# PlasmaControl/spectrogram-enhancement

Hardware: AMD Instinct MI355X
Metric: spectrograms/s (STFT+VAE-denoise fwd) at 1/2/4/8 GPUs; PSNR vs CPU ref (higher is better)
Workload: dtype fp16; 1 GPU; BASELINE config 5 per GPU: end-to-end STFT -> SVD -> autoencoder-denoise inference stream, 16,512-sample fp16 shots -> specgr 128x128 (256 hann / hop 128) -> denoiseSignal default -> 3-layer conv AE (16/32/64, 5x5) fp16 forward -> fp16 reconstructions (32,768 B per shot); shots_per_launch=2048, samples=16512, stft_dtype=fp32, svd_dtype=fp32 (fp64 small algebra), ae_dtype=fp16, parallelism=shot-sharded x1, streams_per_gpu=2

## Files before the change

### spectrogram-enhancement_amd/csrc/conv_rows.hip

```cpp
#include <hip/hip_runtime.h>

#include <algorithm>
#include <cstdint>
#include <string>
#include <type_traits>

#include "lds_dma.hpp"
#include "specenh.h"
#include "runtime.hpp"
#include "wave.hpp"

namespace specenh {

namespace {

typedef _Float16 f16x8 __attribute__((ext_vector_type(8)));
typedef __bf16 bf16x8 __attribute__((ext_vector_type(8)));
typedef float f32x4 __attribute__((ext_vector_type(4)));

template <typename T>
__device__ __forceinline__ f32x4 mfma(const uint4& a, const uint4& b, f32x4 acc) {
  if constexpr (__is_same(T, _Float16))
    return __builtin_amdgcn_mfma_f32_16x16x32_f16(__builtin_bit_cast(f16x8, a),
                                                  __builtin_bit_cast(f16x8, b), acc, 0, 0, 0);
  else
    return __builtin_amdgcn_mfma_f32_16x16x32_bf16(__builtin_bit_cast(bf16x8, a),
                                                   __builtin_bit_cast(bf16x8, b), acc, 0, 0, 0);
}

template <typename T>
__device__ __forceinline__ uint32_t pack2(float lo, float hi) {
  typedef float f2 __attribute__((ext_vector_type(2)));
  typedef T t2 __attribute__((ext_vector_type(2)));
  return __builtin_bit_cast(uint32_t, __builtin_convertvector(f2{lo, hi}, t2));
}


__device__ __forceinline__ float max_pair(float v) {
  const float o = __int_as_float(__builtin_amdgcn_update_dpp(0, __float_as_int(v), 0xB1, 0xF, 0xF, true));
  return fmaxf(v, o);
}

template <int CIN, int COUT, int W, int K = 5>
struct RC {
  static constexpr int NWIN = W / 16;
  static constexpr int NNB = COUT / 16;
  static constexpr int WAVES = NWIN * NNB;
  static constexpr int THREADS = 64 * WAVES;
  static constexpr int PIX = CIN * 2;
  static constexpr int ROWB = (W + 4) * PIX;
  static constexpr int RING = 8;
  static constexpr int LDS = RING * ROWB;
  static constexpr int NW = CIN == 16 ? 13 : K * K;
  static_assert(K == 5 || (CIN == 32 && (K == 3 || K == 5)), "kernel size");
  static constexpr int CPP = CIN / 8;
  static constexpr int CHUNKS = W * CPP;
  static constexpr int WPR = CHUNKS / 64;
  static constexpr int DMA_WAVES = 2 * WPR;
  static_assert(WAVES == 8 && CHUNKS % 64 == 0 && DMA_WAVES <= WAVES, "shape");
  static constexpr int WPE = CIN == 16 || K == 3 ? 4 : 2;
};

struct CRArgs {
  const void* x;
  const void* w;
  const float* b;
  void* out;
  int N, H;
  int lgb;
};

template <typename T, int CIN, int COUT, int W, int K = 5>
__global__ __launch_bounds__((RC<CIN, COUT, W, K>::THREADS))
__attribute__((amdgpu_waves_per_eu(RC<CIN, COUT, W, K>::WPE)))
void conv_rows_pool_kernel(CRArgs a) {
  using C = RC<CIN, COUT, W, K>;
  extern __shared__ __attribute__((aligned(16))) unsigned char ring[];
  const int tid = threadIdx.x, lane = tid & 63;
  const int wv = __builtin_amdgcn_readfirstlane(tid >> 6);
  const int m = lane & 15, kg = lane >> 4;
  const int wx = wv % C::NWIN, nb = wv / C::NWIN;
  const int x0 = 16 * wx;
  const int H = a.H, SPI = H / 2 + 1;
  const int G = gridDim.x;
  const int nimg = ((int)a.N - (int)blockIdx.x + G - 1) / G;
  const int S = nimg * SPI + 1;

  {
    uint4* z = reinterpret_cast<uint4*>(ring);
    for (int e = tid; e < C::LDS / 16; e += C::THREADS) z[e] = uint4{0u, 0u, 0u, 0u};
  }

  uint4 wf[C::NW];
  {
    const T* __restrict__ Wg = reinterpret_cast<const T*>(a.w);
    const int co = 16 * nb + m;
    auto tap = [&](int ky, int kx, int c8) {
      return *reinterpret_cast<const uint4*>(Wg + ((co * K + ky) * K + kx) * CIN + c8);
    };
    if constexpr (CIN == 32) {
#pragma unroll
      for (int t = 0; t < K * K; ++t) wf[t] = tap(t / K, t % K, 8 * kg);
    } else {
      const int hi = kg >> 1, c8 = 8 * (kg & 1);
#pragma unroll
      for (int ky = 0; ky < 5; ++ky) {
        wf[ky] = tap(ky, hi, c8);
        wf[5 + ky] = tap(ky, 2 + hi, c8);
      }
      wf[10] = tap(hi, 4, c8);
      wf[11] = tap(2 + hi, 4, c8);
      wf[12] = hi ? uint4{0u, 0u, 0u, 0u} : tap(4, 4, c8);
    }
  }
  const f32x4 bias = f32x4{a.b[16 * nb + 4 * kg], a.b[16 * nb + 4 * kg + 1],
                           a.b[16 * nb + 4 * kg + 2], a.b[16 * nb + 4 * kg + 3]};

  int boff[CIN == 32 ? K : 1];
  int foff = 0, foffw = 0, fo0 = 0;
  if constexpr (CIN == 32) {
#pragma unroll
    for (int kx = 0; kx < K; ++kx) {
      const int ps = x0 + m + kx + 2 - K / 2;
      boff[kx] = ps * 64 + 16 * (kg ^ ((ps >> 1) & 3));
    }
  } else {
    boff[0] = (x0 + m + (kg >> 1)) * 32 + 16 * (kg & 1);
    const int fo = (x0 + m + 4) * 32 + 16 * (kg & 1);
    fo0 = fo;
    foff = fo + (kg >> 1) * C::ROWB;
    foffw = fo - (kg >> 1) * 7 * C::ROWB;
  }

  const T* __restrict__ X = reinterpret_cast<const T*>(a.x);
  const bool dma_wave = wv < C::DMA_WAVES;
  int dsrc = 0, ddst = 0;
  if (dma_wave) {
    const int c = (wv % C::WPR) * 64 + lane;
    const int ps = 2 + c / C::CPP, gs = c % C::CPP;
    const int g = CIN == 32 ? (gs ^ ((ps >> 1) & 3)) : gs;
    dsrc = (ps - 2) * CIN + 8 * g;
    ddst = 2 * C::PIX + (wv % C::WPR) * 1024;
  }
  auto stage_at = [&](int s, int il, int q) -> bool {
    if (!dma_wave) return false;
    const int r = 2 * q + wv / C::WPR;
    unsigned char* dst = ring + ((2 * s + wv / C::WPR) & 7) * C::ROWB + ddst;
    if (s < S && il < nimg && r < H) {
      const long long n = (long long)blockIdx.x + (long long)il * G;
      lds_dma16_s(X + ((n * H + r) * W) * CIN, 2u * dsrc, dst);
      return true;
    }
    *reinterpret_cast<uint4*>(dst + 16 * lane) = uint4{0u, 0u, 0u, 0u};
    return false;
  };
  auto stage = [&](int s) { return stage_at(s, s / SPI, s - (s / SPI) * SPI); };
  __syncthreads();
  stage(0);
  stage(1);
  stage(2);
  asm volatile("s_waitcnt vmcnt(0)" ::: "memory");
  lds_barrier();

  f32x4 acc[6];
#pragma unroll
  for (int i = 0; i < 6; ++i) acc[i] = bias;
  T* __restrict__ O = reinterpret_cast<T*>(a.out);
  const int PW = W / 2, PHh = H / 2;

  int ilA = -1, qA = SPI - 2, ilC = 0, qC = 0, ilS = 3 / SPI, qS = 3 - (3 / SPI) * SPI;
  auto adv = [&](int& il, int& q) {
    if (++q == SPI) { q = 0; ++il; }
  };
  auto step = [&](auto ic, const int s) {
    constexpr int I = decltype(ic)::value;
    auto slot = [](int d) { return (2 * I + d + 12) % 6; };
    {
      f32x4& r0 = acc[slot(-4)];
      f32x4& r1 = acc[slot(-3)];
      {
        const int il = ilA, q = qA;
        if (il >= 0 && il < nimg && q < PHh) {
          float v[4];
#pragma unroll
          for (int i = 0; i < 4; ++i) v[i] = fmaxf(max_pair(fmaxf(r0[i], r1[i])), 0.f);
          const long long n = (long long)blockIdx.x + (long long)il * G;
          const long long o = ((n * PHh + q) * PW + (x0 + m) / 2) * COUT + 16 * nb + 4 * kg;
          *reinterpret_cast<uint2*>(O + o) = uint2{pack2<T>(v[0], v[1]), pack2<T>(v[2], v[3])};
        }
      }
      r0 = bias;
      r1 = bias;
    }
    const bool issued = stage_at(s + 3, ilS, qS);
    const int il = ilC, q = qC;
    if (il < nimg && 2 * q < H) {
      constexpr int NB = CIN == 32 ? K : 3;
      uint4 bf[2][NB];
#pragma unroll
      for (int j = 0; j < 2; ++j) {
        const int rs = (2 * s + j) & 7;
        const unsigned char* rb = ring + rs * C::ROWB;
        if constexpr (CIN == 32) {
#pragma unroll
          for (int kx = 0; kx < K; ++kx) bf[j][kx] = *reinterpret_cast<const uint4*>(rb + boff[kx]);
        } else {
          bf[j][0] = *reinterpret_cast<const uint4*>(rb + boff[0]);
          bf[j][1] = *reinterpret_cast<const uint4*>(rb + boff[0] + 64);
          bf[j][2] = *reinterpret_cast<const uint4*>(rb + (rs == 7 ? foffw : foff));
        }
      }
      uint4 bT = uint4{0u, 0u, 0u, 0u};
      if constexpr (CIN == 16) {
        if (q == 0) {
          bT = *reinterpret_cast<const uint4*>(ring + ((2 * s) & 7) * C::ROWB + fo0);
          if (kg < 2) bT = uint4{0u, 0u, 0u, 0u};
        }
      }
      __builtin_amdgcn_sched_barrier(0);
#pragma unroll
      for (int j = 0; j < 2; ++j) {
        if constexpr (CIN == 32) {
#pragma unroll
          for (int kx = 0; kx < K; ++kx)
#pragma unroll
            for (int ky = 0; ky < K; ++ky) {
              f32x4& ac = acc[slot(j + K / 2 - ky)];
              ac = mfma<T>(wf[ky * K + kx], bf[j][kx], ac);
            }
        } else {
#pragma unroll
          for (int ky = 0; ky < 5; ++ky) {
            f32x4& ac = acc[slot(j + 2 - ky)];
            ac = mfma<T>(wf[ky], bf[j][0], ac);
          }
#pragma unroll
          for (int ky = 0; ky < 5; ++ky) {
            f32x4& ac = acc[slot(j + 2 - ky)];
            ac = mfma<T>(wf[5 + ky], bf[j][1], ac);
          }
          acc[slot(j + 2)] = mfma<T>(wf[10], bf[j][2], acc[slot(j + 2)]);
          acc[slot(j)] = mfma<T>(wf[11], bf[j][2], acc[slot(j)]);
          acc[slot(j - 2)] = mfma<T>(wf[12], bf[j][2], acc[slot(j - 2)]);
          if (j == 0 && q == 0) acc[slot(1)] = mfma<T>(wf[10], bT, acc[slot(1)]);
        }
      }
    }
    if (issued) asm volatile("s_waitcnt vmcnt(1)" ::: "memory");
    else asm volatile("s_waitcnt vmcnt(0)" ::: "memory");
    adv(ilA, qA);
    adv(ilC, qC);
    adv(ilS, qS);
    lds_barrier();
  };
  int s = 0;
  for (; s + 3 <= S; s += 3) {
    step(std::integral_constant<int, 0>{}, s);
    step(std::integral_constant<int, 1>{}, s + 1);
    step(std::integral_constant<int, 2>{}, s + 2);
  }
  if (s < S) step(std::integral_constant<int, 0>{}, s);
  if (s + 1 < S) step(std::integral_constant<int, 1>{}, s + 1);
}

template <typename T, int CIN, int COUT, int W, int K = 5>
hipError_t launch_rows(const CRArgs& a, hipStream_t st) {
  using C = RC<CIN, COUT, W, K>;
  const void* k = reinterpret_cast<const void*>(&conv_rows_pool_kernel<T, CIN, COUT, W, K>);
  static int per_cu[64] = {};
  int dev = 0;
  hipError_t e = hipGetDevice(&dev);
  if (e != hipSuccess) return e;
  if (dev < 0 || dev >= 64) dev = 0;
  if (per_cu[dev] == 0) {
    int pc = 0;
    e = hipOccupancyMaxActiveBlocksPerMultiprocessor(&pc, k, C::THREADS, C::LDS);
    if (e != hipSuccess) return e;
    per_cu[dev] = std::max(1, pc);
  }
  const long long grid = std::min<long long>(a.N, (long long)per_cu[dev] * device_cus());
  SPECENH_LAUNCH((conv_rows_pool_kernel<T, CIN, COUT, W, K>), dim3((unsigned)grid),
                 dim3(C::THREADS), C::LDS, st, a);
  return hipGetLastError();
}

template <int CO, int W>
struct TC {
  static constexpr int CI = 64;
  static constexpr int NWIN = W / 16, NNB = CO / 16;
  static constexpr int WAVES = NWIN * NNB;
  static constexpr int THREADS = 64 * WAVES;
  static constexpr int ROWB = (W + 2) * CI * 2;
  static constexpr int RING = 8;
  static constexpr int LDS = RING * ROWB;
  static constexpr int DMA_WAVES = W * CI * 2 / 1024;
  static_assert(WAVES == 4 && DMA_WAVES <= WAVES, "shape");
};

__device__ __forceinline__ constexpr int tky(int py, int dy) { return 2 * dy + 3 - py; }
__device__ __forceinline__ constexpr bool ttap(int ph, int dy, int dx) {
  return tky(ph >> 1, dy) >= 0 && tky(ph >> 1, dy) < 5 && tky(ph & 1, dx) >= 0 &&
         tky(ph & 1, dx) < 5;
}

template <typename T>
__device__ __forceinline__ uint32_t relu2(uint32_t p) {
  if constexpr (__is_same(T, _Float16)) {
    typedef _Float16 h2 __attribute__((ext_vector_type(2)));
    const h2 z = h2{(_Float16)0.f, (_Float16)0.f};
    return __builtin_bit_cast(uint32_t, __builtin_elementwise_max(__builtin_bit_cast(h2, p), z));
  } else {
    typedef short s2 __attribute__((ext_vector_type(2)));
    const uint32_t neg = __builtin_bit_cast(uint32_t, __builtin_bit_cast(s2, p) >> (short)15);
    return p & ~neg;
  }
}
template <typename T>
__device__ __forceinline__ uint2 relu_pack4(const f32x4& v) {
  return uint2{relu2<T>(pack2<T>(v[0], v[1])), relu2<T>(pack2<T>(v[2], v[3]))};
}

template <typename T, int CO, int W, int LEAD>
__global__ __launch_bounds__((TC<CO, W>::THREADS)) __attribute__((amdgpu_waves_per_eu(2)))
void convt_rows_kernel(CRArgs a) {
  static_assert(LEAD >= 1 && LEAD <= 4, "8-row ring: positions g .. g + 3 + LEAD live");
  using C = TC<CO, W>;
  extern __shared__ __attribute__((aligned(16))) unsigned char ring[];
  const int tid = threadIdx.x, lane = tid & 63;
  const int wv = __builtin_amdgcn_readfirstlane(tid >> 6);
  const int m = lane & 15, kg = lane >> 4;
  const int wx = wv % C::NWIN, nb = wv / C::NWIN;
  const int H = a.H, lgb = a.lgb, HB = H >> lgb, bmask = (1 << lgb) - 1;
  const int SPI = HB + (lgb ? 2 : 1);
  const int G = gridDim.x;
  const int nimg = (((int)a.N << lgb) - (int)blockIdx.x + G - 1) / G;
  const int S = nimg * SPI;

  {
    uint4* z = reinterpret_cast<uint4*>(ring);
    for (int e = tid; e < C::LDS / 16; e += C::THREADS) z[e] = uint4{0u, 0u, 0u, 0u};
  }
  uint4 wf[50];
  {
    const T* __restrict__ Wg = reinterpret_cast<const T*>(a.w);
    int u = 0;
#pragma unroll
    for (int ph = 0; ph < 4; ++ph)
#pragma unroll
      for (int dy = -1; dy <= 1; ++dy)
#pragma unroll
        for (int dx = -1; dx <= 1; ++dx) {
          if (!ttap(ph, dy, dx)) continue;
#pragma unroll
          for (int kh = 0; kh < 2; ++kh)
            wf[u++] = *reinterpret_cast<const uint4*>(
                Wg + (((16 * nb + m) * 5 + tky(ph >> 1, dy)) * 5 + tky(ph & 1, dx)) * 64 +
                32 * kh + 8 * kg);
        }
  }
  const f32x4 bias = f32x4{a.b[16 * nb + 4 * kg], a.b[16 * nb + 4 * kg + 1],
                           a.b[16 * nb + 4 * kg + 2], a.b[16 * nb + 4 * kg + 3]};
  resident_loads_landed();
  int xo[3];
#pragma unroll
  for (int dx = -1; dx <= 1; ++dx) {
    const int ps = 16 * wx + m + dx + 1;
    xo[dx + 1] = ps * 128 + 16 * (kg ^ (ps & 7));
  }
  const T* __restrict__ X = reinterpret_cast<const T*>(a.x);
  const bool dma_wave = wv < C::DMA_WAVES;
  int dsrc = 0;
  if (dma_wave) {
    const int c = 64 * wv + lane;
    const int ps = 1 + c / 8, gs = c & 7;
    dsrc = (ps - 1) * 64 + 8 * (gs ^ (ps & 7));
  }
  auto stage_at = [&](int p, int il, int q) -> bool {
    if (!dma_wave) return false;
    unsigned char* dst = ring + (p & 7) * C::ROWB + 128 + 1024 * wv;
    const int v = (int)blockIdx.x + il * G;
    const int r = (v & bmask) * HB + q - 1;
    if (il < nimg && r >= 0 && r < H) {
      const long long n = (long long)(v >> lgb);
      lds_dma16_s(X + ((n * H + r) * W) * 64, 2u * dsrc, dst);
      return true;
    }
    *reinterpret_cast<uint4*>(dst + 16 * lane) = uint4{0u, 0u, 0u, 0u};
    return false;
  };
  auto stage = [&](int p) -> bool {
    const int il = p / SPI;
    return stage_at(p, il, p - il * SPI);
  };
  __syncthreads();
#pragma unroll
  for (int p = 0; p < 3 + LEAD; ++p) stage(p);
  asm volatile("s_waitcnt vmcnt(0)" ::: "memory");
  lds_barrier();

  T* __restrict__ O = reinterpret_cast<T*>(a.out);
  const int OW = 2 * W;
  uint2 pk[4];
  long long po = 0;
  bool held = false;
  int vmn = 0;
  int mk[LEAD + 1];
#pragma unroll
  for (int i = 0; i <= LEAD; ++i) mk[i] = -1;
  auto store_held = [&]() {
    if (held) {
#pragma unroll
      for (int ph = 0; ph < 4; ++ph)
        gstore8(O + po + ((ph >> 1) * OW + (ph & 1)) * CO, pk[ph]);
      vmn += 4;
    }
  };
  int il = 0, s = 0;
  int ilp = (3 + LEAD) / SPI, sp = 3 + LEAD - ilp * SPI;
  for (int g = 0; g < S; ++g) {
    store_held();
    held = false;
    mk[LEAD] = stage_at(g + 3 + LEAD, ilp, sp) ? ++vmn : -1;
    if (s < HB) {
      f32x4 acc[4] = {bias, bias, bias, bias};
      int u0[4] = {0, 8, 20, 32};
#pragma unroll
      for (int dy = -1; dy <= 1; ++dy) {
        const unsigned char* src = ring + ((g + 1 + dy) & 7) * C::ROWB;
#pragma unroll
        for (int dx = -1; dx <= 1; ++dx) {
          const uint4 b0 = *reinterpret_cast<const uint4*>(src + xo[dx + 1]);
          const uint4 b1 = *reinterpret_cast<const uint4*>(src + (xo[dx + 1] ^ 64));
#pragma unroll
          for (int ph = 0; ph < 4; ++ph)
// ... 1075 lines not shown
  produce(1, 1 / SPI, 1 % SPI);
  lds_barrier();

  f32x4 acc[6];
#pragma unroll
  for (int i = 0; i < 6; ++i) acc[i] = bias2_ld();
  T* __restrict__ O = reinterpret_cast<T*>(a.out);
  const int PW = 32, PHh = H / 2;
  int c_1 = 0, c_2 = 0;
  auto fdiv = [](int x, int d) { return x >= 0 ? x / d : -((-x + d - 1) / d); };
  int ilA = fdiv(-2, SPI), qA = -2 - ilA * SPI;
  int qC = 0;
  int ilB = 2 / SPI, qB = 2 - ilB * SPI;
  int ilD = (32 + wv) / PPI, rD = 32 + wv - ilD * PPI;
  auto adv = [](int& il, int& q, int by, int per) {
    q += by;
    if (q >= per) { q -= per; ++il; }
  };

  auto step = [&](auto ic, const int s) {
    constexpr int I = decltype(ic)::value;
    auto slot = [](int d) { return (2 * I + d + 12) % 6; };
    int ns = 0;
    {
      f32x4& r0 = acc[slot(-4)];
      f32x4& r1 = acc[slot(-3)];
      {
        const int il = ilA, q = qA;
        if (il >= 0 && il < nimg && q < PHh) {
          ns = 1;
          float v[4];
#pragma unroll
          for (int i = 0; i < 4; ++i) v[i] = fmaxf(max_pair(fmaxf(r0[i], r1[i])), 0.f);
          const long long n = (long long)blockIdx.x + (long long)il * G;
          const long long o = ((n * PHh + q) * PW + (x0 + m) / 2) * 32 + 16 * nb + 4 * kg;
          *reinterpret_cast<uint2*>(O + o) = uint2{pack2<T>(v[0], v[1]), pack2<T>(v[2], v[3])};
        }
      }
      const f32x4 bias = bias2_ld();
      r0 = bias;
      r1 = bias;
    }
    const int nd = wv < 4 ? stage1_at(4 * s + 32 + wv, ilD, rD - 2) : 0;
    shift1(4 * s + 16);
    const int q = qC;
    auto conv2_rows = [&]() {
#pragma unroll
    for (int j = 0; j < 2; ++j) {
      const int rs = (2 * s + j) & 7;
      const unsigned char* rb = ring + rs * C::ROWB;
      const uint4 b0 = *reinterpret_cast<const uint4*>(rb + boff);
      const uint4 b2 = *reinterpret_cast<const uint4*>(rb + boff + 64);
      uint4 bF = *reinterpret_cast<const uint4*>(rb + (rs == 7 ? foffw : foff));
      if (j == 1 && q == SPI - 1) bF = uint4{0u, 0u, 0u, 0u};
#pragma unroll
      for (int ky = 0; ky < 5; ++ky) {
        f32x4& ac = acc[slot(j + 2 - ky)];
        ac = mfma<T>(wf[ky], b0, ac);
      }
#pragma unroll
      for (int ky = 0; ky < 5; ++ky) {
        f32x4& ac = acc[slot(j + 2 - ky)];
        ac = mfma<T>(wf[5 + ky], b2, ac);
      }
      acc[slot(j + 2)] = mfma<T>(wf[10], bF, acc[slot(j + 2)]);
      acc[slot(j)] = mfma<T>(wf[11], bF, acc[slot(j)]);
      acc[slot(j - 2)] = mfma<T>(wf[12], bF, acc[slot(j - 2)]);
      if (j == 0) {
        uint4 bT = *reinterpret_cast<const uint4*>(ring + ((2 * s) & 7) * C::ROWB + fo);
        if (kg < 2 || q != 0) bT = uint4{0u, 0u, 0u, 0u};
        acc[slot(1)] = mfma<T>(wf[10], bT, acc[slot(1)]);
      }
    }
    };
    if (SPECENH_ENC2_STAGGER && wv >= 4) {
      conv2_rows();
      produce(s + 2, ilB, qB);
    } else {
      produce(s + 2, ilB, qB);
      conv2_rows();
    }
    if (wv < 4) {
      const int younger = c_2 + c_1 + ns + nd;
      if (younger >= 6) {
        asm volatile("s_waitcnt vmcnt(6)" ::: "memory");
      } else switch (younger) {
        case 0: asm volatile("s_waitcnt vmcnt(0)" ::: "memory"); break;
        case 1: asm volatile("s_waitcnt vmcnt(1)" ::: "memory"); break;
        case 2: asm volatile("s_waitcnt vmcnt(2)" ::: "memory"); break;
        case 3: asm volatile("s_waitcnt vmcnt(3)" ::: "memory"); break;
        case 4: asm volatile("s_waitcnt vmcnt(4)" ::: "memory"); break;
        case 5: asm volatile("s_waitcnt vmcnt(5)" ::: "memory"); break;
        default: asm volatile("s_waitcnt vmcnt(6)" ::: "memory"); break;
      }
    }
    c_2 = c_1;
    c_1 = ns + nd;
    adv(ilA, qA, 1, SPI);
    qC = qC + 1 == SPI ? 0 : qC + 1;
    adv(ilB, qB, 1, SPI);
    adv(ilD, rD, 4, PPI);
    lds_barrier();
  };
  int s = 0;
  for (; s + 3 <= S; s += 3) {
    step(std::integral_constant<int, 0>{}, s);
    step(std::integral_constant<int, 1>{}, s + 1);
    step(std::integral_constant<int, 2>{}, s + 2);
  }
  if (s < S) step(std::integral_constant<int, 0>{}, s);
  if (s + 1 < S) step(std::integral_constant<int, 1>{}, s + 1);
}

constexpr int E2LDS = RC<16, 32, 64>::LDS + E2RROWS * E2ROW * 4 + 48 * 4;

template <typename T, int WPE>
hipError_t launch_enc2_wpe(const E2Args& a, hipStream_t st) {
  const void* k = reinterpret_cast<const void*>(&enc2_rows_kernel<T, WPE>);
  static int per_cu[64] = {};
  int dev = 0;
  hipError_t e = hipGetDevice(&dev);
  if (e != hipSuccess) return e;
  if (dev < 0 || dev >= 64) dev = 0;
  if (per_cu[dev] == 0) {
    int pc = 0;
    e = hipOccupancyMaxActiveBlocksPerMultiprocessor(&pc, k, 512, E2LDS);
    if (e != hipSuccess) return e;
    per_cu[dev] = std::max(1, pc);
  }
  const long long grid = std::min<long long>(a.N, (long long)per_cu[dev] * device_cus());
  SPECENH_LAUNCH((enc2_rows_kernel<T, WPE>), dim3((unsigned)grid), dim3(512), E2LDS, st, a);
  return hipGetLastError();
}

template <typename T>
hipError_t launch_enc2(const E2Args& a, hipStream_t st) {
  return variant(V_ENC2_WPE2) ? launch_enc2_wpe<T, 2>(a, st) : launch_enc2_wpe<T, 4>(a, st);
}

}

int conv_rows_pool(int dtype, const void* x, int N, int H, int W, int CI, const void* w,
                   const float* b, int CO, int K, void* out, hipStream_t st, bool* launched) {
  *launched = false;
  if (variant(V_CONV_NO_ROWS) != 0 || N <= 0 || H < 2 || (H & 1) || !b) return SPECENH_OK;
  if ((long long)N * H * W * CI >= (1ll << 31)) return SPECENH_OK;
  CRArgs a{};
  a.x = x; a.w = w; a.b = b; a.out = out; a.N = N; a.H = H;
  hipError_t e = hipSuccess;
  const bool f16 = dtype == SPECENH_DTYPE_F16;
  if (dtype != SPECENH_DTYPE_F16 && dtype != SPECENH_DTYPE_BF16) return SPECENH_OK;
  if (CI == 16 && CO == 32 && W == 64 && K == 5)
    e = f16 ? launch_rows<_Float16, 16, 32, 64>(a, st) : launch_rows<__bf16, 16, 32, 64>(a, st);
  else if (CI == 32 && CO == 64 && W == 32 && K == 5)
    e = f16 ? launch_rows<_Float16, 32, 64, 32>(a, st) : launch_rows<__bf16, 32, 64, 32>(a, st);
  else if (CI == 32 && CO == 32 && W == 64 && K == 5)
    e = f16 ? launch_rows<_Float16, 32, 32, 64>(a, st) : launch_rows<__bf16, 32, 32, 64>(a, st);
  else if (CI == 32 && CO == 32 && W == 64 && K == 3)
    e = f16 ? launch_rows<_Float16, 32, 32, 64, 3>(a, st) : launch_rows<__bf16, 32, 32, 64, 3>(a, st);
  else
    return SPECENH_OK;
  if (e != hipSuccess) return set_error(SPECENH_EHIP, std::string("conv_rows: ") + hipGetErrorString(e));
  *launched = true;
  return SPECENH_OK;
}

}

namespace specenh {

int convt_rows(int dtype, const void* x, int N, int H, int W, int CI, const void* w,
               const float* b, int CO, int K, void* out, hipStream_t st, bool* launched) {
  *launched = false;
  if (variant(V_CONVT_NO_ROWS) != 0 || N <= 0 || H <= 0 || !b) return SPECENH_OK;
  if (dtype != SPECENH_DTYPE_F16 && dtype != SPECENH_DTYPE_BF16) return SPECENH_OK;
  if ((long long)N * 4 * H * W * CO >= (1ll << 31)) return SPECENH_OK;
  CRArgs a{};
  a.x = x; a.w = w; a.b = b; a.out = out; a.N = N; a.H = H;
  const bool f16 = dtype == SPECENH_DTYPE_F16;
  hipError_t e;
  if (CI == 32) {
    if (CO != 32 || W != 32) return SPECENH_OK;
    if (K == 3) e = f16 ? launch_convt_rows32<_Float16, 32, 32, 3>(a, st) : launch_convt_rows32<__bf16, 32, 32, 3>(a, st);
    else if (K == 5) e = f16 ? launch_convt_rows32<_Float16, 32, 32, 5>(a, st) : launch_convt_rows32<__bf16, 32, 32, 5>(a, st);
    else if (K == 7) e = f16 ? launch_convt_rows32<_Float16, 32, 32, 7>(a, st) : launch_convt_rows32<__bf16, 32, 32, 7>(a, st);
    else return SPECENH_OK;
    if (e != hipSuccess) return set_error(SPECENH_EHIP, std::string("convt_rows32: ") + hipGetErrorString(e));
    *launched = true;
    return SPECENH_OK;
  }
  if (CI != 64 || K != 5) return SPECENH_OK;
  if (CO == 64 && W == 16 && variant(V_CONVT_SHARED_RING) == 0 && variant(V_CONVT_PG) != 0)
    e = f16 ? launch_convt_rows_pg<_Float16>(a, st) : launch_convt_rows_pg<__bf16>(a, st);
  else if (CO == 64 && W == 16 && variant(V_CONVT_SHARED_RING) == 0 && variant(V_CONVT_STORE8) != 0)
    e = f16 ? launch_convt_rows_pw<_Float16, true>(a, st)
            : launch_convt_rows_pw<__bf16, true>(a, st);
  else if (CO == 64 && W == 16 && variant(V_CONVT_SHARED_RING) == 0)
    e = f16 ? launch_convt_rows_pw<_Float16, false>(a, st)
            : launch_convt_rows_pw<__bf16, false>(a, st);
  else if (CO == 64 && W == 16)
    e = f16 ? launch_convt_rows<_Float16, 64, 16>(a, st) : launch_convt_rows<__bf16, 64, 16>(a, st);
  else if (CO == 32 && W == 32)
    e = f16 ? launch_convt_rows<_Float16, 32, 32>(a, st) : launch_convt_rows<__bf16, 32, 32>(a, st);
  else
    return SPECENH_OK;
  if (e != hipSuccess) return set_error(SPECENH_EHIP, std::string("convt_rows: ") + hipGetErrorString(e));
  *launched = true;
  return SPECENH_OK;
}

}

namespace specenh {

int conv1_rows_pool(int dtype, const void* x, int N, int H, int W, const void* w,
                    const float* b, int CO, void* out, hipStream_t st, bool* launched) {
  *launched = false;
  if (variant(V_CONV1_NO_ROWS) != 0 || N <= 0 || H < 2 || (H & 1) || W != C1W || CO != 16 || !b)
    return SPECENH_OK;
  if (dtype != SPECENH_DTYPE_F16 && dtype != SPECENH_DTYPE_BF16) return SPECENH_OK;
  if (((uintptr_t)x & 15) || (long long)N * H * W >= (1ll << 31)) return SPECENH_OK;
  CRArgs a{};
  a.x = x; a.w = w; a.b = b; a.out = out; a.N = N; a.H = H;
  const hipError_t e = dtype == SPECENH_DTYPE_F16 ? launch_conv1_rows<_Float16>(a, st)
                                                  : launch_conv1_rows<__bf16>(a, st);
  if (e != hipSuccess) return set_error(SPECENH_EHIP, std::string("conv1_rows: ") + hipGetErrorString(e));
  *launched = true;
  return SPECENH_OK;
}

}

extern "C" int specenh_encoder2(int dtype, const void* x, int N, int H, int W, const void* w1_gemm,
                                const float* b1, int CO1, const void* w2_gemm, const float* b2,
                                int CO2, int k, void* out, void* stream) {
  using namespace specenh;
  if (N < 0 || H <= 0 || W <= 0) return set_error(SPECENH_EINVAL, "bad input shape");
  if (dtype != SPECENH_DTYPE_F16 && dtype != SPECENH_DTYPE_BF16)
    return set_error(SPECENH_EUNSUPPORTED, "fused encoder: fp16 / bf16 only");
  if (W != C1W || CO1 != 16 || CO2 != 32 || k != 5 || (H & 3))
    return set_error(SPECENH_EUNSUPPORTED,
                     "fused encoder: Conv2D(16, 5) + pool + Conv2D(32, 5) + pool on 128-wide "
                     "one-channel images, height a multiple of 4");
  if (N == 0) return SPECENH_OK;
  if (!x || !w1_gemm || !b1 || !w2_gemm || !b2 || !out) return set_error(SPECENH_EINVAL, "null pointer");
  if (((uintptr_t)x & 15) || (long long)N * H * W >= (1ll << 31))
    return set_error(SPECENH_EINVAL, "input must be 16-byte aligned and below 2^31 elements");
  E2Args a{};
  a.x = x; a.w1 = w1_gemm; a.b1 = b1; a.w2 = w2_gemm; a.b2 = b2; a.out = out; a.N = N; a.H = H;
  hipStream_t st = (hipStream_t)stream;
  static LdsOptIn lds_site;
  (void)allow_lds(lds_site,
                  {reinterpret_cast<const void*>(&enc2_rows_kernel<_Float16, 4>),
                   reinterpret_cast<const void*>(&enc2_rows_kernel<__bf16, 4>),
                   reinterpret_cast<const void*>(&enc2_rows_kernel<_Float16, 2>),
                   reinterpret_cast<const void*>(&enc2_rows_kernel<__bf16, 2>)},
                  E2LDS);
  const hipError_t e = dtype == SPECENH_DTYPE_F16 ? launch_enc2<_Float16>(a, st)
                                                  : launch_enc2<__bf16>(a, st);
  if (e != hipSuccess) return set_error(SPECENH_EHIP, std::string("encoder2: ") + hipGetErrorString(e));
  return SPECENH_OK;
}
```

### spectrogram-enhancement_amd/csrc/lds_dma.hpp

```cpp
#pragma once

#include <hip/hip_runtime.h>

#include <cstdint>

namespace specenh {

__device__ __forceinline__ void lds_dma16(const void* src, void* dst) {
  const unsigned m0 = (unsigned)(uintptr_t)(__attribute__((address_space(3))) void*)dst;
  asm volatile("s_mov_b32 m0, %1\n\ts_nop 0\n\tglobal_load_lds_dwordx4 %0, off"
               :
               : "v"(src), "s"(m0)
               : "m0");
}

__device__ __forceinline__ void lds_dma16_s(const void* sbase, unsigned voff, void* dst) {
  const unsigned m0 = (unsigned)(uintptr_t)(__attribute__((address_space(3))) void*)dst;
  asm volatile("s_mov_b32 m0, %2\n\ts_nop 0\n\tglobal_load_lds_dwordx4 %0, %1"
               :
               : "v"(voff), "s"(sbase), "s"(m0)
               : "m0");
}

__device__ __forceinline__ void gstore8(void* dst, uint2 v) {
  asm volatile("global_store_dwordx2 %0, %1, off" : : "v"(dst), "v"(v) : "memory");
}

template <int OFF>
__device__ __forceinline__ void gstore16_s(void* sbase, unsigned voff, uint4 v) {
  static_assert(OFF >= 0 && OFF < 4096, "13-bit signed immediate");
  typedef unsigned u32x4 __attribute__((ext_vector_type(4)));
  asm volatile("global_store_dwordx4 %0, %1, %2 offset:%3"
               :
               : "v"(voff), "v"(__builtin_bit_cast(u32x4, v)), "s"(sbase), "n"(OFF)
               : "memory");
}

__device__ __forceinline__ void resident_loads_landed() { __builtin_amdgcn_s_waitcnt(0x0F70); }

__device__ __forceinline__ void wait_vmcnt(int n) {
  switch (__builtin_amdgcn_readfirstlane(n)) {
    case 0: asm volatile("s_waitcnt vmcnt(0)" ::: "memory"); break;
    case 1: asm volatile("s_waitcnt vmcnt(1)" ::: "memory"); break;
    case 2: asm volatile("s_waitcnt vmcnt(2)" ::: "memory"); break;
    case 3: asm volatile("s_waitcnt vmcnt(3)" ::: "memory"); break;
    case 4: asm volatile("s_waitcnt vmcnt(4)" ::: "memory"); break;
    case 5: asm volatile("s_waitcnt vmcnt(5)" ::: "memory"); break;
    case 6: asm volatile("s_waitcnt vmcnt(6)" ::: "memory"); break;
    case 7: asm volatile("s_waitcnt vmcnt(7)" ::: "memory"); break;
    case 8: asm volatile("s_waitcnt vmcnt(8)" ::: "memory"); break;
    case 9: asm volatile("s_waitcnt vmcnt(9)" ::: "memory"); break;
    case 10: asm volatile("s_waitcnt vmcnt(10)" ::: "memory"); break;
    case 11: asm volatile("s_waitcnt vmcnt(11)" ::: "memory"); break;
    case 12: asm volatile("s_waitcnt vmcnt(12)" ::: "memory"); break;
    case 13: asm volatile("s_waitcnt vmcnt(13)" ::: "memory"); break;
    case 14: asm volatile("s_waitcnt vmcnt(14)" ::: "memory"); break;
    default: asm volatile("s_waitcnt vmcnt(15)" ::: "memory"); break;
  }
}

template <int STEADY>
__device__ __forceinline__ void wait_vmcnt_ss(int n) {
  static_assert(STEADY >= 0 && STEADY <= 15, "vmcnt is 4 bits on gfx9");
  if (__builtin_amdgcn_readfirstlane(n) >= STEADY)
    asm volatile("s_waitcnt vmcnt(%0)" ::"n"(STEADY) : "memory");
  else
    wait_vmcnt(n);
}

}
```

### spectrogram-enhancement_amd/csrc/runtime.hip

```cpp
#include "runtime.hpp"

#include <algorithm>
#include <atomic>
#include <cstdlib>
#include <cstring>
#include <mutex>
#include <string>

#include "specenh.h"

namespace specenh {
namespace {

struct VariantName {
  const char* name;
  int dflt;
};
constexpr VariantName kVariants[V_COUNT] = {
    {"CONVT_PAIR", 0},      {"PATCH_NO_WL", 0},      {"PATCH_NO_K5", 0},
    {"PATCH_WSPLIT", -1},   {"CONV_NO_S2", 0},       {"CONV_NO_PATCH", 0},
    {"CONV_NO_C1MFMA", 0},  {"CONV_NO_NARROW", 0},   {"WGRAD_GENERIC", 0},
    {"WGRAD_NO_CO1", 0},    {"WGRAD_PERPHASE", 0},   {"SVD_GRAM_TILES", 0},
    {"TAIL_TILES", 0},      {"DECODER_UNFUSED", 0},  {"SVD_NO_TOP1", 0},
    {"CONV_NO_ROWS", 0},    {"CONVT_NO_ROWS", 0},    {"CONV1_NO_ROWS", 0},
    {"ENCODER_UNFUSED", 0},  {"STFT_NO_HOLD", 0},    {"D3_MAP", 0},
    {"ENC2_WPE2", 0},        {"CONVT_SHARED_RING", 0}, {"SVD_RECON_VALU", 0},
    {"ROWS_SHORT_LEAD", 0},  {"SVD_GRAM_F32", 0},
    {"SVD_RECON_BLOCKS", 0}, {"CONVT_PG", 0}, {"SVD_GZ_ROWS", 0}, {"EIG_SPLIT", 0}, {"CO1_VALU", 0},
    {"C1_MASK_MFMA", 1}, {"S2_MIN_NT", 2}, {"PATCH_MIN_WG", 512}, {"WGRAD_WG", 1024}, {"WGRAD_C1_TILES", 4},
    {"EIG_GRID", 32}, {"ROWS_BANDS", -1}, {"CONVT_STORE8", 0},
};

std::atomic<int> g_variant[V_COUNT];
std::once_flag g_variant_once;

void init_variants() {
  for (int i = 0; i < V_COUNT; ++i) {
    int v = kVariants[i].dflt;
    std::string env = std::string("SPECENH_") + kVariants[i].name;
    if (const char* s = std::getenv(env.c_str()); s && *s) v = std::atoi(s);
    g_variant[i].store(v, std::memory_order_relaxed);
  }
}

int variant_index(const char* name) {
  if (!name) return -1;
  if (std::strncmp(name, "SPECENH_", 8) == 0) name += 8;
  for (int i = 0; i < V_COUNT; ++i)
    if (std::strcmp(name, kVariants[i].name) == 0) return i;
  return -1;
}

constexpr int kMaxDevices = 64;
std::atomic<int> g_cus[kMaxDevices];

constexpr int kRing = 256;
thread_local const void* g_ring[kRing];
thread_local long long g_launches = 0;

thread_local std::string g_last_error;

}

int set_error(int code, const std::string& msg) {
  g_last_error = msg;
  return code;
}

int variant(Variant v) {
  std::call_once(g_variant_once, init_variants);
  return g_variant[v].load(std::memory_order_relaxed);
}

int device_cus() {
  int dev = 0;
  if (hipGetDevice(&dev) != hipSuccess || dev < 0 || dev >= kMaxDevices) return 256;
  int c = g_cus[dev].load(std::memory_order_relaxed);
  if (c > 0) return c;
  if (hipDeviceGetAttribute(&c, hipDeviceAttributeMultiprocessorCount, dev) != hipSuccess || c <= 0)
    c = 256;
  g_cus[dev].store(c, std::memory_order_relaxed);
  return c;
}

hipError_t allow_lds(LdsOptIn& site, std::initializer_list<const void*> kernels, int bytes) {
  static_assert(sizeof(site.done) / sizeof(site.done[0]) == kMaxDevices, "one flag per device");
  int dev = 0;
  hipError_t e = hipGetDevice(&dev);
  if (e != hipSuccess) return e;
  const bool known = dev >= 0 && dev < kMaxDevices;
  if (known && site.done[dev].load(std::memory_order_acquire)) return hipSuccess;
  for (const void* k : kernels) {
    hipFuncAttributes fa{};
    e = hipFuncGetAttributes(&fa, k);
    if (e != hipSuccess) return e;
    e = hipFuncSetAttribute(k, hipFuncAttributeMaxDynamicSharedMemorySize,
                            std::min(bytes, 160 * 1024 - (int)fa.sharedSizeBytes));
    if (e != hipSuccess) return e;
  }
  if (known) site.done[dev].store(true, std::memory_order_release);
  return hipSuccess;
}

void note_launch(const void* kernel) { g_ring[g_launches++ % kRing] = kernel; }

}

extern "C" {

const char* specenh_last_error(void) { return specenh::g_last_error.c_str(); }

int specenh_set_variant(const char* name, int value) {
  const int i = specenh::variant_index(name);
  if (i < 0) return specenh::set_error(SPECENH_EINVAL, std::string("unknown variant ") + (name ? name : "(null)"));
  std::call_once(specenh::g_variant_once, specenh::init_variants);
  specenh::g_variant[i].store(value, std::memory_order_relaxed);
  return SPECENH_OK;
}

int specenh_get_variant(const char* name, int* value) {
  const int i = specenh::variant_index(name);
  if (i < 0 || !value)
    return specenh::set_error(SPECENH_EINVAL, std::string("unknown variant ") + (name ? name : "(null)"));
  *value = specenh::variant((specenh::Variant)i);
  return SPECENH_OK;
}

long long specenh_launch_count(void) { return specenh::g_launches; }

const char* specenh_kernel_name_at(long long index) {
  using namespace specenh;
  if (index < 0 || index >= g_launches || index < g_launches - kRing) return "";
  const char* n = hipKernelNameRefByPtr(g_ring[index % kRing], nullptr);
  return n ? n : "";
}

int specenh_stream_wait(void* waiter, void* signaler, int device_scope) {
  using namespace specenh;
  constexpr int kEvents = 256;
  static std::mutex mu;
  static hipEvent_t ring[kMaxDevices][2][kEvents] = {};
  static int next[kMaxDevices][2] = {};
  int dev = 0, cur = 0;
  if (hipStreamGetDevice((hipStream_t)signaler, &dev) != hipSuccess || dev < 0 ||
      dev >= kMaxDevices || hipGetDevice(&cur) != hipSuccess)
    return set_error(SPECENH_EHIP, "stream_wait: no device for the signaler stream");
  const int kind = device_scope ? 1 : 0;
  hipEvent_t ev;
  {
    std::lock_guard<std::mutex> lk(mu);
    hipEvent_t& e = ring[dev][kind][next[dev][kind]];
    next[dev][kind] = (next[dev][kind] + 1) % kEvents;
    if (!e) {
      const unsigned fl = hipEventDisableTiming | (device_scope ? hipEventDisableSystemFence : 0u);
      const bool sw = cur != dev;
      if (sw && hipSetDevice(dev) != hipSuccess)
        return set_error(SPECENH_EHIP, "stream_wait: hipSetDevice");
      const hipError_t ce = hipEventCreateWithFlags(&e, fl);
      if (sw) (void)hipSetDevice(cur);
      if (ce != hipSuccess) {
        e = nullptr;
        return set_error(SPECENH_EHIP, "stream_wait: hipEventCreateWithFlags");
      }
    }
    ev = e;
  }
  if (hipEventRecord(ev, (hipStream_t)signaler) != hipSuccess ||
      hipStreamWaitEvent((hipStream_t)waiter, ev, 0) != hipSuccess)
    return set_error(SPECENH_EHIP, "stream_wait: record / wait");
  return SPECENH_OK;
}

const char* specenh_last_kernel_name(void) {
  return specenh_kernel_name_at(specenh::g_launches - 1);
}

}
```

### spectrogram-enhancement_amd/csrc/runtime.hpp

```cpp
#pragma once

#include <hip/hip_runtime.h>

#include <atomic>
#include <initializer_list>
#include <string>

namespace specenh {

int set_error(int code, const std::string& msg);

inline int ilog2i(int n) {
  int l = 0;
  while ((1 << l) < n) ++l;
  return l;
}

enum Variant : int {
  V_CONVT_PAIR = 0,
  V_PATCH_NO_WL,
  V_PATCH_NO_K5,
  V_PATCH_WSPLIT,
  V_CONV_NO_S2,
  V_CONV_NO_PATCH,
  V_CONV_NO_C1MFMA,
  V_CONV_NO_NARROW,
  V_WGRAD_GENERIC,
  V_WGRAD_NO_CO1,
  V_WGRAD_PERPHASE,
  V_SVD_GRAM_TILES,
  V_TAIL_TILES,
  V_DECODER_UNFUSED,
  V_SVD_NO_TOP1,
  V_CONV_NO_ROWS,
  V_CONVT_NO_ROWS,
  V_CONV1_NO_ROWS,
  V_ENCODER_UNFUSED,
  V_STFT_NO_HOLD,
  V_D3_MAP,
  V_ENC2_WPE2,
  V_CONVT_SHARED_RING,
  V_SVD_RECON_VALU,
  V_ROWS_SHORT_LEAD,
  V_SVD_GRAM_F32,
  V_SVD_RECON_BLOCKS,
  V_CONVT_PG,
  V_SVD_GZ_ROWS,
  V_EIG_SPLIT,
  V_CO1_VALU,
  V_C1_MASK_MFMA,
  V_S2_MIN_NT,
  V_PATCH_MIN_WG,
  V_WGRAD_WG,
  V_WGRAD_C1_TILES,
  V_EIG_GRID,
  V_ROWS_BANDS,
  V_CONVT_STORE8,
  V_COUNT
};

int variant(Variant v);

int device_cus();

struct LdsOptIn {
  std::atomic<bool> done[64];
};
hipError_t allow_lds(LdsOptIn& site, std::initializer_list<const void*> kernels, int bytes);

void note_launch(const void* kernel);

}

#define SPECENH_LAUNCH(K, ...)                                        \
  do {                                                                \
    ::specenh::note_launch(reinterpret_cast<const void*>(&K));        \
    hipLaunchKernelGGL(K, __VA_ARGS__);                               \
  } while (0)
```

Baseline: 1.978 million spectrograms/s.

## Add software-pipelined schedule for 32->64 conv rows kernel with fragment double-buffering

Adds a SCHED=1 path to the row-streaming conv+pool kernel for the 32->64 channel, width-32 layer, enabled by default through a new variant flag. It double-buffers the LDS B-fragments so the next step's fragment loads overlap the current MFMAs. It also splits the MFMAs around the pool/store, uses scalar-base global stores and loads with pointer increments, and counts outstanding vm ops so it waits only as much as needed. It also adds optional compile-time cycle instrumentation. The cost is more registers for the second fragment buffer, which may lower occupancy, and more complex wait-count logic.

```diff
diff --git a/spectrogram-enhancement_amd/csrc/conv_rows.hip b/spectrogram-enhancement_amd/csrc/conv_rows.hip
--- a/spectrogram-enhancement_amd/csrc/conv_rows.hip
+++ b/spectrogram-enhancement_amd/csrc/conv_rows.hip
@@ -50,6 +50,9 @@
   static constexpr int PIX = CIN * 2;
   static constexpr int ROWB = (W + 4) * PIX;
   static constexpr int RING = 8;
+  static constexpr int LEAD = 3;
+  static constexpr int PF = 1;
+  static_assert(2 * (LEAD + 1) <= RING && PF < LEAD - 1, "ring slots live: steps s - 1 + PF .. s + LEAD");
   static constexpr int LDS = RING * ROWB;
   static constexpr int NW = CIN == 16 ? 13 : K * K;
   static_assert(K == 5 || (CIN == 32 && (K == 3 || K == 5)), "kernel size");
@@ -70,10 +73,41 @@
   int lgb;
 };
 
-template <typename T, int CIN, int COUT, int W, int K = 5>
+#ifdef SPECENH_CR_STATS
+__device__ unsigned long long cr_stats[1024 * 8 * 8];
+struct CRClock {
+  long long last = 0, seg[6] = {0, 0, 0, 0, 0, 0}, n = 0;
+  template <int SEG>
+  __device__ __forceinline__ void mark() {
+    __builtin_amdgcn_sched_barrier(0);
+    asm volatile("s_waitcnt lgkmcnt(0)" ::: "memory");
+    const long long t = __builtin_amdgcn_s_memtime();
+    asm volatile("s_waitcnt lgkmcnt(0)" ::: "memory");
+    __builtin_amdgcn_sched_barrier(0);
+    if constexpr (SEG >= 0) seg[SEG] += t - last;
+    if constexpr (SEG == 5) ++n;
+    last = t;
+  }
+  __device__ void flush(int wv) {
+    if ((threadIdx.x & 63) == 0 && blockIdx.x < 1024) {
+      unsigned long long* p = cr_stats + (blockIdx.x * 8 + wv) * 8;
+#pragma unroll
+      for (int i = 0; i < 6; ++i) p[i] = seg[i];
+      p[6] = n;
+      p[7] = 0;
+    }
+  }
+};
+#define CR_MARK(SEG) clk.mark<SEG>()
+#else
+#define CR_MARK(SEG) ((void)0)
+#endif
+
+template <typename T, int CIN, int COUT, int W, int K = 5, int SCHED = 0>
 __global__ __launch_bounds__((RC<CIN, COUT, W, K>::THREADS))
 __attribute__((amdgpu_waves_per_eu(RC<CIN, COUT, W, K>::WPE)))
 void conv_rows_pool_kernel(CRArgs a) {
+  static_assert(SCHED == 0 || (SCHED == 1 && CIN == 32), "schedule");
   using C = RC<CIN, COUT, W, K>;
   extern __shared__ __attribute__((aligned(16))) unsigned char ring[];
   const int tid = threadIdx.x, lane = tid & 63;
@@ -172,6 +206,151 @@
   auto adv = [&](int& il, int& q) {
     if (++q == SPI) { q = 0; ++il; }
   };
+#ifdef SPECENH_CR_STATS
+  CRClock clk;
+#endif
+  if constexpr (SCHED == 1) {
+    static_assert(C::PF == 1, "two fragment buffers");
+    uint4 bf[2][2][K];
+    auto frags = [&](auto pc, auto jc, const int t) {
+      constexpr int P = decltype(pc)::value, j = decltype(jc)::value;
+      const unsigned char* rb = ring + (((2 * t) & 7) + j) * C::ROWB;
+#pragma unroll
+      for (int kx = 0; kx < K; ++kx) bf[P][j][kx] = *reinterpret_cast<const uint4*>(rb + boff[kx]);
+    };
+    using I0 = std::integral_constant<int, 0>;
+    using I1 = std::integral_constant<int, 1>;
+    frags(I0{}, I0{}, 0);
+    frags(I0{}, I1{}, 0);
+    resident_loads_landed();
+    constexpr long long ROWO = (long long)(W / 2) * COUT * (long long)sizeof(T);
+    const unsigned ovo = (unsigned)((((x0 + m) / 2) * COUT + 16 * nb + 4 * kg) * (int)sizeof(T));
+    unsigned char* ob = reinterpret_cast<unsigned char*>(a.out) +
+                        (((long long)blockIdx.x - G) * PHh + qA) * ROWO;
+    const long long ojump = (long long)(G - 1) * PHh * ROWO;
+    constexpr long long ROWX = (long long)W * CIN * (long long)sizeof(T);
+    const unsigned char* xs = reinterpret_cast<const unsigned char*>(a.x) +
+        (((long long)blockIdx.x + (long long)ilS * G) * H + 2 * qS + wv / C::WPR) * ROWX;
+    const long long xjump = (long long)(G - 1) * H * ROWX;
+    int vmn = 0;
+    int mk0 = -1, mk1 = -1;
+    auto lt = [](int x, int y) -> unsigned { return (unsigned)(x - y) >> 31; };
+    const int nimgs = __builtin_amdgcn_readfirstlane(nimg);
+    ilS = __builtin_amdgcn_readfirstlane(ilS);
+    qS = __builtin_amdgcn_readfirstlane(qS);
+    auto flags = [&]() -> unsigned {
+      return (lt(ilC, nimgs) & lt(2 * qC, H)) | ((lt(-1, ilA) & lt(ilA, nimgs) & lt(qA, PHh)) << 1) |
+             ((lt(ilS, nimgs) & lt(2 * qS, H)) << 2);
+    };
+    unsigned fl = __builtin_amdgcn_readfirstlane(flags());
+    auto next = [&]() {
+      if (++qA == SPI) { qA = 0; ++ilA; ob += ojump; } else { ob += ROWO; }
+      adv(ilC, qC);
+      if (++qS == SPI) { qS = 0; ++ilS; xs += xjump; } else { xs += 2 * ROWX; }
+      fl = __builtin_amdgcn_readfirstlane(flags());
+      asm volatile("" : "+s"(fl));
+    };
+    auto step1 = [&](auto ic, const int s) {
+      constexpr int I = decltype(ic)::value % 3, P = decltype(ic)::value & 1;
+      auto slot = [](int d) { return (2 * I + d + 12) % 6; };
+      using PN = std::integral_constant<int, P ^ 1>;
+      mk1 = -1;
+      if (dma_wave) {
+        unsigned char* dst = ring + ((2 * (s + C::LEAD) + wv / C::WPR) & 7) * C::ROWB + ddst;
+        if (fl & 4u) {
+          lds_dma16_s(xs, 2u * dsrc, dst);
+          mk1 = ++vmn;
+        } else {
+          *reinterpret_cast<uint4*>(dst + 16 * lane) = uint4{0u, 0u, 0u, 0u};
+        }
+      }
+      CR_MARK(1);
+      f32x4& r0 = acc[slot(-4)];
+      f32x4& r1 = acc[slot(-3)];
+      const bool pst = (fl & 2u) != 0;
+      auto pool = [&]() {
+        float v[4];
+#pragma unroll
+        for (int i = 0; i < 4; ++i) v[i] = fmaxf(max_pair(fmaxf(r0[i], r1[i])), 0.f);
+        r0 = bias;
+        r1 = bias;
+        return uint2{pack2<T>(v[0], v[1]), pack2<T>(v[2], v[3])};
+      };
+      auto store = [&](const uint2 pk) {
+        if (pst) {
+          gstore8_s(ob, ovo, pk);
+          ++vmn;
+        }
+      };
+      auto mm = [&](int j, int kx, int ky) {
+        f32x4& ac = acc[slot(j + K / 2 - ky)];
+        ac = mfma<T>(wf[ky * K + kx], bf[P][j][kx], ac);
+      };
+      if (fl & 1u) {
+#pragma unroll
+        for (int kx = 0; kx < K; ++kx)
+#pragma unroll
+          for (int ky = 0; ky < K; ++ky)
+            if (K / 2 - ky <= 1) mm(0, kx, ky);
+        const uint2 pk = pool();
+        frags(PN{}, I0{}, s + 1);
+        store(pk);
+        next();
+        frags(PN{}, I1{}, s + 1);
+        asm volatile("" ::: "memory");
+#pragma unroll
+        for (int kx = 0; kx < K; ++kx) {
+#pragma unroll
+          for (int ky = 0; ky < K; ++ky)
+            if (K / 2 - ky > 1) mm(0, kx, ky);
+#pragma unroll
+          for (int ky = 0; ky < K; ++ky)
+            if (1 + K / 2 - ky <= 1) mm(1, kx, ky);
+        }
+#pragma unroll
+        for (int kx = 0; kx < K; ++kx)
+#pragma unroll
+          for (int ky = 0; ky < K; ++ky)
+            if (1 + K / 2 - ky > 1) mm(1, kx, ky);
+      } else {
+        store(pool());
+        next();
+        frags(PN{}, I0{}, s + 1);
+        frags(PN{}, I1{}, s + 1);
+      }
+      CR_MARK(3);
+      if (mk0 >= 0) {
+        const int younger = vmn - mk0;
+        if (younger >= 3) asm volatile("s_waitcnt vmcnt(3)" ::: "memory");
+        else if (younger == 2) asm volatile("s_waitcnt vmcnt(2)" ::: "memory");
+        else if (younger == 1) asm volatile("s_waitcnt vmcnt(1)" ::: "memory");
+        else asm volatile("s_waitcnt vmcnt(0)" ::: "memory");
+      }
+      mk0 = mk1;
+      CR_MARK(4);
+      lds_barrier();
+      CR_MARK(5);
+    };
+    CR_MARK(-1);
+    int s = 0;
+    for (; s + 6 <= S; s += 6) {
+      step1(std::integral_constant<int, 0>{}, s);
+      step1(std::integral_constant<int, 1>{}, s + 1);
+      step1(std::integral_constant<int, 2>{}, s + 2);
+      step1(std::integral_constant<int, 3>{}, s + 3);
+      step1(std::integral_constant<int, 4>{}, s + 4);
+      step1(std::integral_constant<int, 5>{}, s + 5);
+    }
+    if (s < S) step1(std::integral_constant<int, 0>{}, s);
+    if (s + 1 < S) step1(std::integral_constant<int, 1>{}, s + 1);
+    if (s + 2 < S) step1(std::integral_constant<int, 2>{}, s + 2);
+    if (s + 3 < S) step1(std::integral_constant<int, 3>{}, s + 3);
+    if (s + 4 < S) step1(std::integral_constant<int, 4>{}, s + 4);
+#ifdef SPECENH_CR_STATS
+    clk.flush(wv);
+#endif
+    return;
+  }
   auto step = [&](auto ic, const int s) {
     constexpr int I = decltype(ic)::value;
     auto slot = [](int d) { return (2 * I + d + 12) % 6; };
@@ -192,7 +371,9 @@
       r0 = bias;
       r1 = bias;
     }
-    const bool issued = stage_at(s + 3, ilS, qS);
+    CR_MARK(0);
+    const bool issued = stage_at(s + C::LEAD, ilS, qS);
+    CR_MARK(1);
     const int il = ilC, q = qC;
     if (il < nimg && 2 * q < H) {
       constexpr int NB = CIN == 32 ? K : 3;
@@ -217,6 +398,7 @@
           if (kg < 2) bT = uint4{0u, 0u, 0u, 0u};
         }
       }
+      CR_MARK(2);
       __builtin_amdgcn_sched_barrier(0);
 #pragma unroll
       for (int j = 0; j < 2; ++j) {
@@ -246,13 +428,17 @@
         }
       }
     }
+    CR_MARK(3);
     if (issued) asm volatile("s_waitcnt vmcnt(1)" ::: "memory");
     else asm volatile("s_waitcnt vmcnt(0)" ::: "memory");
+    CR_MARK(4);
     adv(ilA, qA);
     adv(ilC, qC);
     adv(ilS, qS);
     lds_barrier();
-  };
+    CR_MARK(5);
+  };
+  CR_MARK(-1);
   int s = 0;
   for (; s + 3 <= S; s += 3) {
     step(std::integral_constant<int, 0>{}, s);
@@ -261,12 +447,15 @@
   }
   if (s < S) step(std::integral_constant<int, 0>{}, s);
   if (s + 1 < S) step(std::integral_constant<int, 1>{}, s + 1);
-}
-
-template <typename T, int CIN, int COUT, int W, int K = 5>
+#ifdef SPECENH_CR_STATS
+  clk.flush(wv);
+#endif
+}
+
+template <typename T, int CIN, int COUT, int W, int K = 5, int SCHED = 0>
 hipError_t launch_rows(const CRArgs& a, hipStream_t st) {
   using C = RC<CIN, COUT, W, K>;
-  const void* k = reinterpret_cast<const void*>(&conv_rows_pool_kernel<T, CIN, COUT, W, K>);
+  const void* k = reinterpret_cast<const void*>(&conv_rows_pool_kernel<T, CIN, COUT, W, K, SCHED>);
   static int per_cu[64] = {};
   int dev = 0;
   hipError_t e = hipGetDevice(&dev);
@@ -279,7 +468,7 @@
     per_cu[dev] = std::max(1, pc);
   }
   const long long grid = std::min<long long>(a.N, (long long)per_cu[dev] * device_cus());
-  SPECENH_LAUNCH((conv_rows_pool_kernel<T, CIN, COUT, W, K>), dim3((unsigned)grid),
+  SPECENH_LAUNCH((conv_rows_pool_kernel<T, CIN, COUT, W, K, SCHED>), dim3((unsigned)grid),
                  dim3(C::THREADS), C::LDS, st, a);
   return hipGetLastError();
 }
@@ -1661,6 +1850,8 @@
   if (dtype != SPECENH_DTYPE_F16 && dtype != SPECENH_DTYPE_BF16) return SPECENH_OK;
   if (CI == 16 && CO == 32 && W == 64 && K == 5)
     e = f16 ? launch_rows<_Float16, 16, 32, 64>(a, st) : launch_rows<__bf16, 16, 32, 64>(a, st);
+  else if (CI == 32 && CO == 64 && W == 32 && K == 5 && variant(V_CONV_ROWS_SCHED) != 0)
+    e = f16 ? launch_rows<_Float16, 32, 64, 32, 5, 1>(a, st) : launch_rows<__bf16, 32, 64, 32, 5, 1>(a, st);
   else if (CI == 32 && CO == 64 && W == 32 && K == 5)
     e = f16 ? launch_rows<_Float16, 32, 64, 32>(a, st) : launch_rows<__bf16, 32, 64, 32>(a, st);
   else if (CI == 32 && CO == 32 && W == 64 && K == 5)
@@ -1770,3 +1961,9 @@
   if (e != hipSuccess) return set_error(SPECENH_EHIP, std::string("encoder2: ") + hipGetErrorString(e));
   return SPECENH_OK;
 }
+
+#ifdef SPECENH_CR_STATS
+extern "C" int specenh_cr_stats(void* host, int bytes) {
+  return hipMemcpyFromSymbol(host, HIP_SYMBOL(specenh::cr_stats), bytes) == hipSuccess ? 0 : -1;
+}
+#endif
diff --git a/spectrogram-enhancement_amd/csrc/lds_dma.hpp b/spectrogram-enhancement_amd/csrc/lds_dma.hpp
--- a/spectrogram-enhancement_amd/csrc/lds_dma.hpp
+++ b/spectrogram-enhancement_amd/csrc/lds_dma.hpp
@@ -24,6 +24,14 @@
 
 __device__ __forceinline__ void gstore8(void* dst, uint2 v) {
   asm volatile("global_store_dwordx2 %0, %1, off" : : "v"(dst), "v"(v) : "memory");
+}
+
+__device__ __forceinline__ void gstore8_s(void* sbase, unsigned voff, uint2 v) {
+  typedef unsigned u32x2 __attribute__((ext_vector_type(2)));
+  asm volatile("global_store_dwordx2 %0, %1, %2"
+               :
+               : "v"(voff), "v"(__builtin_bit_cast(u32x2, v)), "s"(sbase)
+               : "memory");
 }
 
 template <int OFF>
diff --git a/spectrogram-enhancement_amd/csrc/runtime.hip b/spectrogram-enhancement_amd/csrc/runtime.hip
--- a/spectrogram-enhancement_amd/csrc/runtime.hip
+++ b/spectrogram-enhancement_amd/csrc/runtime.hip
@@ -29,6 +29,7 @@
     {"SVD_RECON_BLOCKS", 0}, {"CONVT_PG", 0}, {"SVD_GZ_ROWS", 0}, {"EIG_SPLIT", 0}, {"CO1_VALU", 0},
     {"C1_MASK_MFMA", 1}, {"S2_MIN_NT", 2}, {"PATCH_MIN_WG", 512}, {"WGRAD_WG", 1024}, {"WGRAD_C1_TILES", 4},
     {"EIG_GRID", 32}, {"ROWS_BANDS", -1}, {"CONVT_STORE8", 0},
+    {"CONV_ROWS_SCHED", 1},
 };
 
 std::atomic<int> g_variant[V_COUNT];
diff --git a/spectrogram-enhancement_amd/csrc/runtime.hpp b/spectrogram-enhancement_amd/csrc/runtime.hpp
--- a/spectrogram-enhancement_amd/csrc/runtime.hpp
+++ b/spectrogram-enhancement_amd/csrc/runtime.hpp
@@ -56,6 +56,7 @@
   V_EIG_GRID,
   V_ROWS_BANDS,
   V_CONVT_STORE8,
+  V_CONV_ROWS_SCHED,
   V_COUNT
 };
 
```

Result: faster. 1.998 million spectrograms/s, median of 6 (+1.1%).
